# GatorSense/HyperPRI

Hardware: AMD Instinct MI355X
Metric: HSI cubes/sec (608x968x238) fwd+bwd (higher is better)
Workload: dtype f32; 1 GPU; CubeNET-64 n_channels=238 HSI 608x968 fp32, per-GPU batch 2, train mode, BCEWithLogits, fwd+bwd; global_batch=2, parallelism=dp1

## Files before the change

### hyperpri_amd/csrc/elementwise.hip

```cpp
#include "common.h"

static inline int ew_blocks(long long total) {
  long long b = (total + 255) / 256;
  if (b > 8192) b = 8192;
  if (b < 1) b = 1;
  return (int)b;
}

__global__ void nchw_to_nhwc_kernel(const float* __restrict__ src, float* __restrict__ dst, int C, long long P,
                                    int cs, int coff, int Cw) {
  __shared__ float tile[32][65];
  const int n = blockIdx.z;
  const long long p0 = (long long)blockIdx.x * 64;
  const int c0 = blockIdx.y * 32;
  const int tx = threadIdx.x & 63, ty = threadIdx.x >> 6;
  for (int r = ty; r < 32; r += 4) {
    const int c = c0 + r;
    const long long p = p0 + tx;
    tile[r][tx] = (c < C && p < P) ? src[((long long)n * C + c) * P + p] : 0.f;
  }
  __syncthreads();
  const int cx = threadIdx.x & 31, py = threadIdx.x >> 5;
  for (int r = py; r < 64; r += 8) {
    const long long p = p0 + r;
    const int c = c0 + cx;
    if (p < P && c < Cw) dst[((long long)n * P + p) * cs + coff + c] = tile[cx][r];
  }
}

__global__ __launch_bounds__(256) void nchw_to_nhwc_v4_kernel(const float* __restrict__ src, float* __restrict__ dst, int C,
                                                              long long P, int cs, int coff, int Cw, PlaneOut pl) {
  __shared__ float tile[128][65];
  const int n = blockIdx.z;
  const long long p0 = (long long)blockIdx.x * 128;
  const int c0 = blockIdx.y * 64;
  const int tx = threadIdx.x & 31, ty = threadIdx.x >> 5;
#pragma unroll
  for (int r = ty; r < 64; r += 8) {
    const int c = c0 + r;
    const long long p = p0 + tx * 4;
    f32x4 v = {0.f, 0.f, 0.f, 0.f};
    if (c < C && p < P) v = *reinterpret_cast<const f32x4*>(src + ((long long)n * C + c) * P + p);
    const int rc = (r + (tx >> 3)) & 63;
    tile[tx * 4 + 0][rc] = v[0]; tile[tx * 4 + 1][rc] = v[1]; tile[tx * 4 + 2][rc] = v[2]; tile[tx * 4 + 3][rc] = v[3];
  }
  __syncthreads();
  const int cq = threadIdx.x & 15, py = threadIdx.x >> 4;
#pragma unroll
  for (int r = py; r < 128; r += 16) {
    const long long p = p0 + r;
    const int c = c0 + cq * 4;
    if (p < P && (c < Cw || c < pl.cw)) {
      const int ro = r >> 5;
      f32x4 v = {tile[r][(cq * 4 + 0 + ro) & 63], tile[r][(cq * 4 + 1 + ro) & 63], tile[r][(cq * 4 + 2 + ro) & 63],
                 tile[r][(cq * 4 + 3 + ro) & 63]};
      if (dst != nullptr && c < Cw) *reinterpret_cast<f32x4*>(dst + ((long long)n * P + p) * cs + coff + c) = v;
      if (c < pl.cw) plane_store4(pl, (size_t)((long long)n * P + p), c, v[0], v[1], v[2], v[3]);
    }
  }
}

__global__ void nhwc_to_nchw_kernel(const float* __restrict__ src, float* __restrict__ dst, int C, long long P,
                                    int cs, int coff, int accumulate) {
  __shared__ float tile[64][33];
  const int n = blockIdx.z;
  const long long p0 = (long long)blockIdx.x * 64;
  const int c0 = blockIdx.y * 32;
  const int cx = threadIdx.x & 31, py = threadIdx.x >> 5;
  for (int r = py; r < 64; r += 8) {
    const long long p = p0 + r;
    const int c = c0 + cx;
    tile[r][cx] = (p < P && c < C) ? src[((long long)n * P + p) * cs + coff + c] : 0.f;
  }
  __syncthreads();
  const int tx = threadIdx.x & 63, ty = threadIdx.x >> 6;
  for (int r = ty; r < 32; r += 4) {
    const int c = c0 + r;
    const long long p = p0 + tx;
    if (c < C && p < P) {
      float* o = dst + ((long long)n * C + c) * P + p;
      *o = accumulate ? *o + tile[tx][r] : tile[tx][r];
    }
  }
}

template <bool B16>
__device__ __forceinline__ float4 ew_load4(const float* __restrict__ p) {
  if (B16) {
    const bf16x4_t v = *reinterpret_cast<const bf16x4_t*>(p);
    return make_float4((float)v[0], (float)v[1], (float)v[2], (float)v[3]);
  }
  return *reinterpret_cast<const float4*>(p);
}
template <bool B16>
__device__ __forceinline__ void ew_store4(float* __restrict__ p, float4 v) {
  if (B16) {
    bf16x4_t h;
    h[0] = (h16_t)v.x; h[1] = (h16_t)v.y; h[2] = (h16_t)v.z; h[3] = (h16_t)v.w;
    *reinterpret_cast<bf16x4_t*>(p) = h;
  } else {
    *reinterpret_cast<float4*>(p) = v;
  }
}
template <bool B16>
__device__ __forceinline__ const float* ew_at(const float* base, long long idx) {
  return B16 ? reinterpret_cast<const float*>(reinterpret_cast<const h16_t*>(base) + idx) : base + idx;
}
template <bool B16>
__device__ __forceinline__ float* ew_at(float* base, long long idx) {
  return B16 ? reinterpret_cast<float*>(reinterpret_cast<h16_t*>(base) + idx) : base + idx;
}

template <bool XB>
__global__ void maxpool2_fwd_kernel(const float* __restrict__ x, int x_cs, int x_coff, float* __restrict__ y, int y_cs,
                                    int y_coff, int N, int H, int W, int OH, int OW, int C4v, int C4, PlaneOut pl) {
  const long long total = (long long)N * OH * OW * C4;
  for (long long i = (long long)blockIdx.x * blockDim.x + threadIdx.x; i < total; i += (long long)gridDim.x * blockDim.x) {
    const int c = (int)(i % C4) * 4;
    long long r = i / C4;
    const int ox = (int)(r % OW); r /= OW;
    const int oy = (int)(r % OH);
    const int n = (int)(r / OH);
    const size_t opix = (size_t)(((long long)n * OH + oy) * OW + ox);
    if (c >= C4v * 4) { plane_store4(pl, opix, c, 0.f, 0.f, 0.f, 0.f); continue; }
    const long long b = (((long long)n * H + 2 * oy) * W + 2 * ox) * x_cs + x_coff + c;
    const float4 v00 = ew_load4<XB>(ew_at<XB>(x, b));
    const float4 v01 = ew_load4<XB>(ew_at<XB>(x, b + x_cs));
    const float4 v10 = ew_load4<XB>(ew_at<XB>(x, b + (long long)W * x_cs));
    const float4 v11 = ew_load4<XB>(ew_at<XB>(x, b + (long long)W * x_cs + x_cs));
    float4 m;
    m.x = fmaxf(fmaxf(v00.x, v01.x), fmaxf(v10.x, v11.x));
    m.y = fmaxf(fmaxf(v00.y, v01.y), fmaxf(v10.y, v11.y));
    m.z = fmaxf(fmaxf(v00.z, v01.z), fmaxf(v10.z, v11.z));
    m.w = fmaxf(fmaxf(v00.w, v01.w), fmaxf(v10.w, v11.w));
    if (y != nullptr) *reinterpret_cast<float4*>(y + opix * y_cs + y_coff + c) = m;
    if (pl.p != nullptr) plane_store4(pl, opix, c, m.x, m.y, m.z, m.w);
  }
}

__device__ __forceinline__ int first_argmax4(float a, float b, float c, float d) {
  int k = 0; float m = a;
  if (b > m) { m = b; k = 1; }
  if (c > m) { m = c; k = 2; }
  if (d > m) { k = 3; }
  return k;
}

template <bool XB, bool DXB>
__global__ void maxpool2_bwd_kernel(const float* __restrict__ x, int x_cs, int x_coff, const float* __restrict__ dy,
                                    int dy_cs, int dy_coff, float* __restrict__ dx, int dx_cs, int dx_coff, int N, int H,
                                    int W, int OH, int OW, int C4, int accumulate) {
  const int WH = (H + 1) >> 1, WW = (W + 1) >> 1;
  const unsigned total = (unsigned)N * WH * WW * C4;
  for (unsigned i = blockIdx.x * blockDim.x + threadIdx.x; i < total; i += gridDim.x * blockDim.x) {
    const unsigned c = (i % (unsigned)C4) * 4u;
    unsigned r = i / (unsigned)C4;
    const int wx = (int)(r % (unsigned)WW); r /= (unsigned)WW;
    const int wy = (int)(r % (unsigned)WH);
    const int n = (int)(r / (unsigned)WH);
    const int iy = 2 * wy, ix = 2 * wx;
    const bool row1 = iy + 1 < H, col1 = ix + 1 < W, pooled = wy < OH && wx < OW;
    const long long pix = ((long long)n * H + iy) * W + ix;
    float4 o[4] = {make_float4(0.f, 0.f, 0.f, 0.f), make_float4(0.f, 0.f, 0.f, 0.f), make_float4(0.f, 0.f, 0.f, 0.f),
                   make_float4(0.f, 0.f, 0.f, 0.f)};
    if (pooled) {
      const long long b = pix * x_cs + x_coff + c;
      const float4 v00 = ew_load4<XB>(ew_at<XB>(x, b));
      const float4 v01 = ew_load4<XB>(ew_at<XB>(x, b + x_cs));
      const float4 v10 = ew_load4<XB>(ew_at<XB>(x, b + (long long)W * x_cs));
      const float4 v11 = ew_load4<XB>(ew_at<XB>(x, b + (long long)W * x_cs + x_cs));
      const float4 g = *reinterpret_cast<const float4*>(dy + (((long long)n * OH + wy) * OW + wx) * dy_cs + dy_coff + c);
      const int kx = first_argmax4(v00.x, v01.x, v10.x, v11.x), ky = first_argmax4(v00.y, v01.y, v10.y, v11.y);
      const int kz = first_argmax4(v00.z, v01.z, v10.z, v11.z), kw = first_argmax4(v00.w, v01.w, v10.w, v11.w);
#pragma unroll
      for (int m = 0; m < 4; ++m) {
        o[m].x = kx == m ? g.x : 0.f; o[m].y = ky == m ? g.y : 0.f; o[m].z = kz == m ? g.z : 0.f; o[m].w = kw == m ? g.w : 0.f;
      }
    }
    const long long p = pix * dx_cs + dx_coff + c;
    float* pm[4] = {ew_at<DXB>(dx, p), ew_at<DXB>(dx, p + dx_cs), ew_at<DXB>(dx, p + (long long)W * dx_cs),
                    ew_at<DXB>(dx, p + (long long)W * dx_cs + dx_cs)};
    const bool ok[4] = {true, col1, row1, row1 && col1};
    if (accumulate) {
      float4 old[4];
#pragma unroll
      for (int m = 0; m < 4; ++m) old[m] = ok[m] ? ew_load4<DXB>(pm[m]) : make_float4(0.f, 0.f, 0.f, 0.f);
#pragma unroll
      for (int m = 0; m < 4; ++m) { o[m].x += old[m].x; o[m].y += old[m].y; o[m].z += old[m].z; o[m].w += old[m].w; }
    }
#pragma unroll
    for (int m = 0; m < 4; ++m)
      if (ok[m]) ew_store4<DXB>(pm[m], o[m]);
  }
}

__global__ void copy_slice_kernel(const float* __restrict__ s, int s_cs, int s_coff, float* __restrict__ d, int d_cs,
                                  int d_coff, long long P, int C4, int accumulate) {
  const long long total = P * C4;
  for (long long i = (long long)blockIdx.x * blockDim.x + threadIdx.x; i < total; i += (long long)gridDim.x * blockDim.x) {
    const long long p = i / C4;
    const int c = (int)(i - p * C4) * 4;
    float4 v = *reinterpret_cast<const float4*>(s + p * s_cs + s_coff + c);
    float* o = d + p * d_cs + d_coff + c;
    if (accumulate) {
      const float4 w = *reinterpret_cast<const float4*>(o);
      v.x += w.x; v.y += w.y; v.z += w.z; v.w += w.w;
    }
    *reinterpret_cast<float4*>(o) = v;
  }
}

__global__ void fill_pad_kernel(float* __restrict__ d, int cs, int coff, int N, int H, int W, int C4, int y0, int y1,
                                int x0, int x1) {
  const long long total = (long long)N * H * W * C4;
  for (long long i = (long long)blockIdx.x * blockDim.x + threadIdx.x; i < total; i += (long long)gridDim.x * blockDim.x) {
    const int c = (int)(i % C4) * 4;
    long long r = i / C4;
    const int ix = (int)(r % W); r /= W;
    const int iy = (int)(r % H);
    if (iy >= y0 && iy < y1 && ix >= x0 && ix < x1) continue;
    *reinterpret_cast<float4*>(d + (i / C4) * cs + coff + c) = make_float4(0.f, 0.f, 0.f, 0.f);
  }
}

__global__ void shift_copy_kernel(const float* __restrict__ s, int s_cs, int s_coff, int Hs, int Ws, float* __restrict__ d,
                                  int d_cs, int d_coff, int N, int Hd, int Wd, int oy, int ox, int C4, int accumulate) {
  const long long total = (long long)N * Hd * Wd * C4;
  for (long long i = (long long)blockIdx.x * blockDim.x + threadIdx.x; i < total; i += (long long)gridDim.x * blockDim.x) {
    const int c = (int)(i % C4) * 4;
    long long r = i / C4;
    const int ix = (int)(r % Wd); r /= Wd;
    const int iy = (int)(r % Hd);
    const int n = (int)(r / Hd);
    const int sy = iy - oy, sx = ix - ox;
    float4 v = make_float4(0.f, 0.f, 0.f, 0.f);
    if (sy >= 0 && sy < Hs && sx >= 0 && sx < Ws)
      v = *reinterpret_cast<const float4*>(s + (((long long)n * Hs + sy) * Ws + sx) * s_cs + s_coff + c);
    float* o = d + (i / C4) * d_cs + d_coff + c;
    if (accumulate) {
      const float4 w = *reinterpret_cast<const float4*>(o);
      v.x += w.x; v.y += w.y; v.z += w.z; v.w += w.w;
    }
    *reinterpret_cast<float4*>(o) = v;
  }
}

__global__ void fill_kernel(float* __restrict__ d, long long n, float v) {
  for (long long i = (long long)blockIdx.x * blockDim.x + threadIdx.x; i < n; i += (long long)gridDim.x * blockDim.x) d[i] = v;
}

typedef h16_t bf16x8 __attribute__((ext_vector_type(8)));
__device__ __forceinline__ float oc_bce_elem(float x, float y) { return fmaxf(x, 0.f) - x * y + log1pf(expf(-fabsf(x))); }
__device__ __forceinline__ float oc_bce_grad(float xi, float yi) {
  const float e = expf(-fabsf(xi)), r = 1.f / (1.f + e);
  const float sp = xi >= 0.f ? r : e * r, sn = xi >= 0.f ? e * r : r;
  return (1.f - yi) * sp - yi * sn;
}

template <bool XB>
__device__ __forceinline__ float4 oc_load4(const float* __restrict__ x, size_t idx) {
  if (XB) {
    const bf16x4_t v = *reinterpret_cast<const bf16x4_t*>(reinterpret_cast<const h16_t*>(x) + idx);
    return make_float4((float)v[0], (float)v[1], (float)v[2], (float)v[3]);
  }
  return *reinterpret_cast<const float4*>(x + idx);
}

template <bool BCE, bool XB>
__global__ __launch_bounds__(256) void outconv_fwd_kernel(const float* __restrict__ x, int x_cs, int x_coff, const float* __restrict__ w,
                                   const float* __restrict__ b, float* __restrict__ y, int N, long long P, int C, int K,
                                   const float* __restrict__ target, double* __restrict__ partial) {
  __shared__ double bred[256];
  double bsum = 0.0;
  const int gl = threadIdx.x & 15;
  const long long grp = ((long long)blockIdx.x * blockDim.x + threadIdx.x) >> 4;
  const long long ngrp = ((long long)gridDim.x * blockDim.x) >> 4;
  const int C4 = (C + 3) >> 2;
  if (!XB && K == 1 && (C & 3) == 0 && C4 <= 64) {
    float4 wq[4];
    int qi[4];
#pragma unroll
    for (int j = 0; j < 4; ++j) {
      const int q = gl + 16 * j;
      qi[j] = min(q, C4 - 1) * 4;
      wq[j] = q < C4 ? *reinterpret_cast<const float4*>(w + q * 4) : make_float4(0.f, 0.f, 0.f, 0.f);
    }
    const int nj = (C4 + 15) >> 4;
    const float b0 = b ? b[0] : 0.f;
    const long long NP = (long long)N * P;
    for (long long pg0 = grp; pg0 < NP; pg0 += 4 * ngrp) {
      float4 v[4][4];
#pragma unroll
      for (int u = 0; u < 4; ++u) {
        const long long pg = min(pg0 + u * ngrp, NP - 1);
        const float* xp = x + pg * x_cs + x_coff;
#pragma unroll
        for (int j = 0; j < 4; ++j)
          if (j < nj) v[u][j] = *reinterpret_cast<const float4*>(xp + qi[j]);
      }
      float mine = 0.f;
#pragma unroll
      for (int u = 0; u < 4; ++u) {
        float s = 0.f;
#pragma unroll
        for (int j = 0; j < 4; ++j)
          if (j < nj) { s += v[u][j].x * wq[j].x; s += v[u][j].y * wq[j].y; s += v[u][j].z * wq[j].z; s += v[u][j].w * wq[j].w; }
        s += __shfl_xor(s, 8, 16); s += __shfl_xor(s, 4, 16); s += __shfl_xor(s, 2, 16); s += __shfl_xor(s, 1, 16);
        if (gl == u) mine = s;
      }
      const long long pgm = pg0 + gl * ngrp;
      if (gl < 4 && pgm < NP) {
        const float o = mine + b0;
        y[pgm] = o;
        if (BCE) bsum += (double)oc_bce_elem(o, target[pgm]);
      }
    }
  } else
  for (long long pg = grp; pg < (long long)N * P; pg += ngrp) {
    for (int k = 0; k < K; ++k) {
      float s = 0.f;
      for (int q = gl; q < C4; q += 16) {
        const float4 v = oc_load4<XB>(x, (size_t)pg * x_cs + x_coff + q * 4);
        const float* wk = w + (long long)k * C + q * 4;
        s += v.x * wk[0];
        if (q * 4 + 1 < C) s += v.y * wk[1];
        if (q * 4 + 2 < C) s += v.z * wk[2];
        if (q * 4 + 3 < C) s += v.w * wk[3];
      }
      s += __shfl_xor(s, 8, 16); s += __shfl_xor(s, 4, 16); s += __shfl_xor(s, 2, 16); s += __shfl_xor(s, 1, 16);
      if (gl == 0) {
        const long long n = pg / P, p = pg - n * P;
        const float v = s + (b ? b[k] : 0.f);
        y[(n * K + k) * P + p] = v;
        if (BCE) bsum += (double)oc_bce_elem(v, target[(n * K + k) * P + p]);
      }
    }
  }
  if (BCE) {
    bred[threadIdx.x] = bsum;
    __syncthreads();
    for (int wd = 128; wd > 0; wd >>= 1) {
      if (threadIdx.x < wd) bred[threadIdx.x] += bred[threadIdx.x + wd];
      __syncthreads();
    }
    if (threadIdx.x == 0) partial[blockIdx.x] = bred[0];
  }
}

__device__ __forceinline__ float oc_mul_then_add(float a, float b, float s) {
#pragma clang fp contract(off)
  const float p = a * b;
  return s + p;
}

template <bool BCE, int NJ>
__global__ __launch_bounds__(256) void bn_outconv_fwd_kernel(const float* __restrict__ x, int x_cs, int x_coff, const float* __restrict__ scale,
                                                             const float* __restrict__ shift, int relu, const float* __restrict__ w,
                                                             const float* __restrict__ b, float* __restrict__ y, long long NP, int C,
                                                             const float* __restrict__ target, double* __restrict__ partial) {
  __shared__ double bred[256];
  double bsum = 0.0;
// ... 356 lines not shown
#pragma unroll
    for (int u = 0; u < UF; ++u) add(g[u], xv[u]);
  }
  for (; p < p1; p += rows) {
    float g = dy[p];
    if (BCE) g = oc_bce_grad(g, target[p]) * gs;
    const float4 xq = live ? *reinterpret_cast<const float4*>(x + p * x_cs + x_coff + c) : make_float4(0.f, 0.f, 0.f, 0.f);
    add(g, xq);
  }
  red[0][threadIdx.x] = make_float4(s1[0], s1[1], s1[2], s1[3]);
  red[1][threadIdx.x] = make_float4(s2[0], s2[1], s2[2], s2[3]);
  red[2][threadIdx.x] = make_float4(sw[0], sw[1], sw[2], sw[3]);
  redb[threadIdx.x] = sb;
  __syncthreads();
  if (pr == 0) {
    float4 t1 = make_float4(0.f, 0.f, 0.f, 0.f), t2 = t1, t3 = t1;
    float tb = 0.f;
    for (int r = 0; r < rows; ++r) {
      const float4 a = red[0][r * CQ + cq], b = red[1][r * CQ + cq], d = red[2][r * CQ + cq];
      t1.x += a.x; t1.y += a.y; t1.z += a.z; t1.w += a.w;
      t2.x += b.x; t2.y += b.y; t2.z += b.z; t2.w += b.w;
      t3.x += d.x; t3.y += d.y; t3.z += d.z; t3.w += d.w;
      tb += redb[r * CQ + cq];
    }
    float* o = bnpart + ((size_t)blockIdx.x * 2) * Cpart + c;
    *reinterpret_cast<float4*>(o) = t1;
    *reinterpret_cast<float4*>(o + Cpart) = t2;
    float* h = hwpart + ((size_t)blockIdx.x * 2) * Cpart;
    *reinterpret_cast<float4*>(h + c) = t3;
    if (blockIdx.y == 0 && cq == 0) h[Cpart] = tb;
  }
}

template <bool BCE>
__global__ __launch_bounds__(256) void bn_head_apply_kernel(const float* __restrict__ dy, const float* __restrict__ target,
                                                            const float* __restrict__ gscale, float lscale, const float* __restrict__ x,
                                                            int x_cs, int x_coff, const float* __restrict__ w, float* __restrict__ dx,
                                                            int dx_cs, int dx_coff, const float* __restrict__ mean,
                                                            const float* __restrict__ invstd, const float* __restrict__ scale,
                                                            const float* __restrict__ shift, const float* __restrict__ sums, int NP, int C,
                                                            int Cw, int CQ, int relu, int use_batch_stats, float* __restrict__ dxpart,
                                                            int Cpart) {
  const float gs = BCE ? (gscale ? gscale[0] : 1.f) / (float)((double)NP) * lscale : 1.f;
  __shared__ float4 red[256];
  const int rows = 256 / CQ;
  const int cq = threadIdx.x % CQ, pr = threadIdx.x / CQ;
  const int c = (blockIdx.y * CQ + cq) * 4;
  const bool live = c < Cw;
  float acc[4] = {0.f, 0.f, 0.f, 0.f};
  const float inv_np = 1.f / (float)NP;
  float sc[4], sh[4], mu[4], is[4], k1[4], k2[4], wv[4];
#pragma unroll
  for (int j = 0; j < 4; ++j) {
    const bool ok = c + j < C;
    sc[j] = ok ? scale[c + j] : 0.f;
    sh[j] = ok ? shift[c + j] : 0.f;
    mu[j] = ok ? mean[c + j] : 0.f;
    is[j] = ok ? invstd[c + j] : 0.f;
    wv[j] = ok ? w[c + j] : 0.f;
    k1[j] = (ok && use_batch_stats) ? sums[c + j] * inv_np : 0.f;
    k2[j] = (ok && use_batch_stats) ? sums[C + c + j] * inv_np : 0.f;
  }
  auto put = [&](long long q, float gl, const float4& xq) {
    const float xx[4] = {xq.x, xq.y, xq.z, xq.w};
    float o[4];
#pragma unroll
    for (int j = 0; j < 4; ++j) {
      const float gv = 0.f + gl * wv[j];
      const float gj = (!relu || (xx[j] * sc[j] + sh[j] > 0.f)) ? gv : 0.f;
      const float xh = (xx[j] - mu[j]) * is[j];
      o[j] = (c + j < C) ? sc[j] * (gj - k1[j] - xh * k2[j]) : 0.f;
      acc[j] += o[j];
    }
    *reinterpret_cast<float4*>(dx + (size_t)q * dx_cs + dx_coff + c) = make_float4(o[0], o[1], o[2], o[3]);
  };
  const long long per = ((long long)NP + gridDim.x - 1) / gridDim.x;
  const long long q0 = (long long)blockIdx.x * per;
  const long long q1 = (q0 + per < NP) ? q0 + per : NP;
  long long q = q0 + pr;
  for (; q + 3 * rows < q1; q += 4 * rows) {
    float g[4];
    float4 xv[4];
#pragma unroll
    for (int u = 0; u < 4; ++u) {
      const long long pg = q + u * rows;
      g[u] = dy[pg];
      if (BCE && CQ < 4) g[u] = oc_bce_grad(g[u], target[pg]) * gs;
      xv[u] = live ? *reinterpret_cast<const float4*>(x + (size_t)pg * x_cs + x_coff + c) : make_float4(0.f, 0.f, 0.f, 0.f);
    }
    if (BCE && CQ >= 4) {
      float lg = 0.f, lt = 0.f;
#pragma unroll
      for (int u = 0; u < 4; ++u)
        if (cq == u) { lg = g[u]; lt = target[q + u * rows]; }
      const float mine = oc_bce_grad(lg, lt) * gs;
#pragma unroll
      for (int u = 0; u < 4; ++u) g[u] = __shfl(mine, (threadIdx.x & 63 & ~(CQ - 1)) + u, 64);
    }
    if (live) {
#pragma unroll
      for (int u = 0; u < 4; ++u) put(q + u * rows, g[u], xv[u]);
    }
  }
  if (live)
    for (; q < q1; q += rows) {
      float g = dy[q];
      if (BCE) g = oc_bce_grad(g, target[q]) * gs;
      put(q, g, *reinterpret_cast<const float4*>(x + (size_t)q * x_cs + x_coff + c));
    }
  if (dxpart != nullptr) {
    red[threadIdx.x] = make_float4(acc[0], acc[1], acc[2], acc[3]);
    __syncthreads();
    if (pr == 0 && c < Cpart) {
      float4 t = make_float4(0.f, 0.f, 0.f, 0.f);
      for (int r = 0; r < rows; ++r) { const float4 a = red[r * CQ + cq]; t.x += a.x; t.y += a.y; t.z += a.z; t.w += a.w; }
      float* o = dxpart + ((size_t)blockIdx.x * 2) * Cpart + c;
      *reinterpret_cast<float4*>(o) = t;
      *reinterpret_cast<float4*>(o + Cpart) = make_float4(0.f, 0.f, 0.f, 0.f);
    }
  }
}

template <bool APPLY>
__global__ __launch_bounds__(256) void bn_pool_bwd_kernel(const float* __restrict__ dskip, int ds_cs, int ds_coff,
                                                          const float* __restrict__ dpool, int dp_cs, int dp_coff,
                                                          const float* __restrict__ x, int x_cs, int x_coff, float* __restrict__ dx,
                                                          int dx_cs, int dx_coff, const float* __restrict__ mean,
                                                          const float* __restrict__ invstd, const float* __restrict__ scale,
                                                          const float* __restrict__ shift, const float* __restrict__ sums, int N, int H,
                                                          int W, int C, int Cw, int CQ, float* __restrict__ part, int Cpart) {
  __shared__ float4 red[2][256];
  const int rows = 256 / CQ;
  const int cq = threadIdx.x % CQ, pr = threadIdx.x / CQ;
  const int c = (blockIdx.y * CQ + cq) * 4;
  const int WH = (H + 1) >> 1, WW = (W + 1) >> 1, OH = H >> 1, OW = W >> 1;
  const unsigned nwin = (unsigned)N * WH * WW;
  const unsigned per = (nwin + gridDim.x - 1) / gridDim.x;
  const unsigned w0 = blockIdx.x * per;
  const unsigned w1 = min(nwin, w0 + per);
  float s1[4] = {0.f, 0.f, 0.f, 0.f}, s2[4] = {0.f, 0.f, 0.f, 0.f};
  if (c < (APPLY ? Cw : C)) {
    const float inv_np = 1.f / (float)(N * H * W);
    float sc[4], sh[4], mu[4], is[4], k1[4], k2[4];
#pragma unroll
    for (int j = 0; j < 4; ++j) {
      const bool ok = c + j < C;
      sc[j] = ok ? scale[c + j] : 0.f;
      sh[j] = ok ? shift[c + j] : 0.f;
      mu[j] = ok ? mean[c + j] : 0.f;
      is[j] = ok ? invstd[c + j] : 0.f;
      k1[j] = (ok && APPLY) ? sums[c + j] * inv_np : 0.f;
      k2[j] = (ok && APPLY) ? sums[C + c + j] * inv_np : 0.f;
    }
    for (unsigned wi = w0 + pr; wi < w1; wi += rows) {
      const int wx = (int)(wi % (unsigned)WW);
      const unsigned r = wi / (unsigned)WW;
      const int wy = (int)(r % (unsigned)WH), n = (int)(r / (unsigned)WH);
      const int iy = 2 * wy, ix = 2 * wx;
      const bool row1 = iy + 1 < H, col1 = ix + 1 < W, pooled = wy < OH && wx < OW;
      const long long pix = ((long long)n * H + iy) * W + ix;
#define HPRI_WIN_OK(m_) ((((m_) & 1) == 0 || col1) && (((m_) >> 1) == 0 || row1))
#define HPRI_WIN_PIX(m_) (pix + ((m_) & 1) + (long long)((m_) >> 1) * W)
      float4 xv[4], dv[4];
#pragma unroll
      for (int m = 0; m < 4; ++m) {
        xv[m] = HPRI_WIN_OK(m) ? *reinterpret_cast<const float4*>(x + HPRI_WIN_PIX(m) * x_cs + x_coff + c) : make_float4(0.f, 0.f, 0.f, 0.f);
        dv[m] = (dskip != nullptr && HPRI_WIN_OK(m)) ? *reinterpret_cast<const float4*>(dskip + HPRI_WIN_PIX(m) * ds_cs + ds_coff + c) : make_float4(0.f, 0.f, 0.f, 0.f);
      }
      const float4 gp = pooled ? *reinterpret_cast<const float4*>(dpool + (((long long)n * OH + wy) * OW + wx) * dp_cs + dp_coff + c) : make_float4(0.f, 0.f, 0.f, 0.f);
      const float gq[4] = {gp.x, gp.y, gp.z, gp.w};
      float xx[4][4], dd[4][4], o[4][4];
#pragma unroll
      for (int m = 0; m < 4; ++m) {
        xx[m][0] = xv[m].x; xx[m][1] = xv[m].y; xx[m][2] = xv[m].z; xx[m][3] = xv[m].w;
        dd[m][0] = dv[m].x; dd[m][1] = dv[m].y; dd[m][2] = dv[m].z; dd[m][3] = dv[m].w;
      }
#pragma unroll
      for (int j = 0; j < 4; ++j) {
        float y[4];
#pragma unroll
        for (int m = 0; m < 4; ++m) y[m] = (c + j < C) ? fmaxf(xx[m][j] * sc[j] + sh[j], 0.f) : 0.f;
        const int k = first_argmax4(y[0], y[1], y[2], y[3]);
#pragma unroll
        for (int m = 0; m < 4; ++m) {
          float g = (pooled && k == m) ? gq[j] : 0.f;
          if (dskip != nullptr) g += dd[m][j];
          const float gj = (y[m] > 0.f) ? g : 0.f;
          const float xh = (xx[m][j] - mu[j]) * is[j];
          if (APPLY) {
            o[m][j] = (c + j < C) ? sc[j] * (gj - k1[j] - xh * k2[j]) : 0.f;
          } else if (HPRI_WIN_OK(m)) {
            s1[j] += gj;
            s2[j] += gj * xh;
          }
        }
      }
      if (APPLY) {
#pragma unroll
        for (int m = 0; m < 4; ++m)
          if (HPRI_WIN_OK(m)) *reinterpret_cast<float4*>(dx + HPRI_WIN_PIX(m) * dx_cs + dx_coff + c) = make_float4(o[m][0], o[m][1], o[m][2], o[m][3]);
      }
#undef HPRI_WIN_OK
#undef HPRI_WIN_PIX
    }
  }
  if (!APPLY) {
    red[0][threadIdx.x] = make_float4(s1[0], s1[1], s1[2], s1[3]);
    red[1][threadIdx.x] = make_float4(s2[0], s2[1], s2[2], s2[3]);
    __syncthreads();
    if (pr == 0 && c < Cpart) {
      float4 t1 = make_float4(0.f, 0.f, 0.f, 0.f), t2 = t1;
      for (int r = 0; r < rows; ++r) {
        const float4 a = red[0][r * CQ + cq], b = red[1][r * CQ + cq];
        t1.x += a.x; t1.y += a.y; t1.z += a.z; t1.w += a.w;
        t2.x += b.x; t2.y += b.y; t2.z += b.z; t2.w += b.w;
      }
      float* o = part + ((size_t)blockIdx.x * 2) * Cpart + c;
      *reinterpret_cast<float4*>(o) = t1;
      *reinterpret_cast<float4*>(o + Cpart) = t2;
    }
  }
}

__global__ __launch_bounds__(256) void bn_apply_relu_pool_kernel(const float* __restrict__ x, int x_cs, int x_coff, float* __restrict__ y,
                                                                 int y_cs, int y_coff, float* __restrict__ pool, int p_cs, int p_coff,
                                                                 const float* __restrict__ scale, const float* __restrict__ shift, int N,
                                                                 int H, int W, int C, int C4, int relu) {
  const int WH = (H + 1) >> 1, WW = (W + 1) >> 1, OH = H >> 1, OW = W >> 1;
  const unsigned total = (unsigned)N * WH * WW * C4;
  for (unsigned i = blockIdx.x * blockDim.x + threadIdx.x; i < total; i += gridDim.x * blockDim.x) {
    const int c = (int)(i % (unsigned)C4) * 4;
    unsigned r = i / (unsigned)C4;
    const int wx = (int)(r % (unsigned)WW); r /= (unsigned)WW;
    const int wy = (int)(r % (unsigned)WH);
    const int n = (int)(r / (unsigned)WH);
    const int iy = 2 * wy, ix = 2 * wx;
    const bool row1 = iy + 1 < H, col1 = ix + 1 < W, pooled = wy < OH && wx < OW;
    const long long pix = ((long long)n * H + iy) * W + ix;
    float sc[4], sh[4];
#pragma unroll
    for (int j = 0; j < 4; ++j) {
      const bool ok = c + j < C;
      sc[j] = ok ? scale[c + j] : 0.f;
      sh[j] = ok ? shift[c + j] : 0.f;
    }
    float4 v[4], o[4];
#pragma unroll
    for (int m = 0; m < 4; ++m) {
      const bool okm = ((m & 1) == 0 || col1) && ((m >> 1) == 0 || row1);
      v[m] = okm ? *reinterpret_cast<const float4*>(x + (pix + (m & 1) + (long long)(m >> 1) * W) * x_cs + x_coff + c) : make_float4(0.f, 0.f, 0.f, 0.f);
    }
#pragma unroll
    for (int m = 0; m < 4; ++m) {
      o[m].x = (c + 0 < C) ? v[m].x * sc[0] + sh[0] : 0.f; o[m].y = (c + 1 < C) ? v[m].y * sc[1] + sh[1] : 0.f;
      o[m].z = (c + 2 < C) ? v[m].z * sc[2] + sh[2] : 0.f; o[m].w = (c + 3 < C) ? v[m].w * sc[3] + sh[3] : 0.f;
      if (relu) { o[m].x = fmaxf(o[m].x, 0.f); o[m].y = fmaxf(o[m].y, 0.f); o[m].z = fmaxf(o[m].z, 0.f); o[m].w = fmaxf(o[m].w, 0.f); }
      const bool okm = ((m & 1) == 0 || col1) && ((m >> 1) == 0 || row1);
      if (okm) *reinterpret_cast<float4*>(y + (pix + (m & 1) + (long long)(m >> 1) * W) * y_cs + y_coff + c) = o[m];
    }
    if (pooled) {
      float4 mx;
      mx.x = fmaxf(fmaxf(o[0].x, o[1].x), fmaxf(o[2].x, o[3].x));
      mx.y = fmaxf(fmaxf(o[0].y, o[1].y), fmaxf(o[2].y, o[3].y));
      mx.z = fmaxf(fmaxf(o[0].z, o[1].z), fmaxf(o[2].z, o[3].z));
      mx.w = fmaxf(fmaxf(o[0].w, o[1].w), fmaxf(o[2].w, o[3].w));
      *reinterpret_cast<float4*>(pool + (((long long)n * OH + wy) * OW + wx) * p_cs + p_coff + c) = mx;
    }
  }
}

__device__ __forceinline__ float synth_u(unsigned long long seed, unsigned long long idx) {
  unsigned long long z = seed * 0x9E3779B97F4A7C15ull + idx;
  z ^= z >> 30; z *= 0xBF58476D1CE4E5B9ull;
  z ^= z >> 27; z *= 0x94D049BB133111EBull;
  z ^= z >> 31;
  return (float)(z >> 40) * (1.0f / 16777216.0f);
}

__global__ void synth_kernel(float* __restrict__ d, long long n, unsigned long long seed, int mode, float thr, float scale) {
  for (long long i = (long long)blockIdx.x * blockDim.x + threadIdx.x; i < n; i += (long long)gridDim.x * blockDim.x) {
    const float u = synth_u(seed, (unsigned long long)i);
    d[i] = mode == 0 ? u : (mode == 1 ? (u > thr ? 1.f : 0.f) : (2.f * u - 1.f) * scale);
  }
}

extern "C" int hpri_nchw_to_nhwc_pl(const float* src, float* dst, int N, int C, long long P, int cs, int coff, int Cw,
                                    void* planes, long long plane_stride, int pl_cs, int pl_coff, int pl_cw, int npl,
                                    hipStream_t stream);
extern "C" int hpri_maxpool2_fwd_pl(const float* x, int x_cs, int x_coff, float* y, int y_cs, int y_coff, int N, int H,
                                    int W, int C, void* planes, long long plane_stride, int pl_cs, int pl_coff, int pl_cw,
                                    int npl, hipStream_t stream);
extern "C" int hpri_nchw_to_nhwc(const float* src, float* dst, int N, int C, long long P, int cs, int coff, int Cw,
                                 hipStream_t stream) {
  return hpri_nchw_to_nhwc_pl(src, dst, N, C, P, cs, coff, Cw, nullptr, 0, 0, 0, 0, 0, stream);
}

extern "C" int hpri_nchw_to_nhwc_pl(const float* src, float* dst, int N, int C, long long P, int cs, int coff, int Cw,
                                    void* planes, long long plane_stride, int pl_cs, int pl_coff, int pl_cw, int npl,
                                    hipStream_t stream) {
  HPRI_REQUIRE(src && (dst || planes) && N > 0 && C > 0 && P > 0 && Cw >= C && Cw + coff <= cs, "nchw_to_nhwc: bad arguments");
  PlaneOut po;
  { const int rc_ = hpri_plane_out(&po, planes, plane_stride, pl_cs, pl_coff, pl_cw, npl, C); if (rc_ != HPRI_OK) return rc_; }
  if (P % 4 == 0 && cs % 4 == 0 && coff % 4 == 0 && Cw % 4 == 0 && ((uintptr_t)src & 15) == 0 && ((uintptr_t)dst & 15) == 0) {
    dim3 grid4((unsigned)hpri_cdiv64(P, 128), (unsigned)hpri_cdiv(Cw > po.cw ? Cw : po.cw, 64), (unsigned)N);
    hipLaunchKernelGGL(nchw_to_nhwc_v4_kernel, grid4, dim3(256), 0, stream, src, dst, C, P, cs, coff, Cw, po);
    HPRI_CHECK_LAUNCH();
    return HPRI_OK;
  }
  if (planes != nullptr || dst == nullptr) return hpri_set_error(HPRI_ERR_UNSUPPORTED, "nchw_to_nhwc_pl: plane output needs the 16-byte aligned form");
  dim3 grid((unsigned)hpri_cdiv64(P, 64), (unsigned)hpri_cdiv(Cw, 32), (unsigned)N);
  hipLaunchKernelGGL(nchw_to_nhwc_kernel, grid, dim3(256), 0, stream, src, dst, C, P, cs, coff, Cw);
  HPRI_CHECK_LAUNCH();
  return HPRI_OK;
}

extern "C" int hpri_nhwc_to_nchw(const float* src, float* dst, int N, int C, long long P, int cs, int coff,
                                 int accumulate, hipStream_t stream) {
  HPRI_REQUIRE(src && dst && N > 0 && C > 0 && P > 0 && C + coff <= cs, "nhwc_to_nchw: bad arguments");
  dim3 grid((unsigned)hpri_cdiv64(P, 64), (unsigned)hpri_cdiv(C, 32), (unsigned)N);
  hipLaunchKernelGGL(nhwc_to_nchw_kernel, grid, dim3(256), 0, stream, src, dst, C, P, cs, coff, accumulate);
  HPRI_CHECK_LAUNCH();
  return HPRI_OK;
}

#define HPRI_REQ_V4(cs, coff) HPRI_REQUIRE((cs) % 4 == 0 && (coff) % 4 == 0, "channel stride/offset must be multiples of 4")

extern "C" int hpri_maxpool2_fwd(const float* x, int x_cs, int x_coff, float* y, int y_cs, int y_coff, int N, int H,
                                 int W, int C, hipStream_t stream) {
  return hpri_maxpool2_fwd_pl(x, x_cs, x_coff, y, y_cs, y_coff, N, H, W, C, nullptr, 0, 0, 0, 0, 0, stream);
}

template <bool XB>
static int maxpool2_fwd_impl(const float* x, int x_cs, int x_coff, float* y, int y_cs, int y_coff, int N, int H,
                             int W, int C, void* planes, long long plane_stride, int pl_cs, int pl_coff, int pl_cw,
                             int npl, hipStream_t stream) {
  HPRI_REQUIRE(x && (y || planes) && N > 0 && H >= 2 && W >= 2 && C > 0 && C % 4 == 0, "maxpool2_fwd: bad arguments");
  HPRI_REQ_V4(x_cs, x_coff);
  if (y != nullptr) { HPRI_REQ_V4(y_cs, y_coff); }
  PlaneOut po;
  { const int rc_ = hpri_plane_out(&po, planes, plane_stride, pl_cs, pl_coff, pl_cw, npl, C); if (rc_ != HPRI_OK) return rc_; }
  const int OH = H / 2, OW = W / 2;
  const int c4 = (C > po.cw ? C : po.cw) / 4;
  hipLaunchKernelGGL(maxpool2_fwd_kernel<XB>, dim3(ew_blocks((long long)N * OH * OW * c4)), dim3(256), 0, stream, x, x_cs,
                     x_coff, y, y_cs, y_coff, N, H, W, OH, OW, C / 4, c4, po);
  HPRI_CHECK_LAUNCH();
  return HPRI_OK;
}

extern "C" int hpri_maxpool2_fwd_pl(const float* x, int x_cs, int x_coff, float* y, int y_cs, int y_coff, int N, int H,
                                    int W, int C, void* planes, long long plane_stride, int pl_cs, int pl_coff, int pl_cw,
                                    int npl, hipStream_t stream) {
  HPRI_REQUIRE(y != nullptr, "maxpool2_fwd: bad arguments");
  return maxpool2_fwd_impl<false>(x, x_cs, x_coff, y, y_cs, y_coff, N, H, W, C, planes, plane_stride, pl_cs, pl_coff, pl_cw, npl, stream);
}

extern "C" int hpri_maxpool2_fwd_x16(const void* x16, int x_cs, int x_coff, float* y, int y_cs, int y_coff, int N, int H,
                                     int W, int C, void* planes, long long plane_stride, int pl_cs, int pl_coff, int pl_cw,
                                     int npl, hipStream_t stream) {
  return maxpool2_fwd_impl<true>(reinterpret_cast<const float*>(x16), x_cs, x_coff, y, y_cs, y_coff, N, H, W, C, planes, plane_stride,
                                 pl_cs, pl_coff, pl_cw, npl, stream);
}

extern "C" int hpri_maxpool2_bwd(const float* x, int x_cs, int x_coff, const float* dy, int dy_cs, int dy_coff, float* dx,
                                 int dx_cs, int dx_coff, int N, int H, int W, int C, int accumulate, hipStream_t stream) {
  HPRI_REQUIRE(x && dy && dx && N > 0 && H >= 2 && W >= 2 && C > 0 && C % 4 == 0, "maxpool2_bwd: bad arguments");
  HPRI_REQ_V4(x_cs, x_coff); HPRI_REQ_V4(dy_cs, dy_coff); HPRI_REQ_V4(dx_cs, dx_coff);
  const long long windows = (long long)N * ((H + 1) / 2) * ((W + 1) / 2) * (C / 4);
  HPRI_REQUIRE(windows < (1ll << 31), "maxpool2_bwd: more than 2^31 window quads");
  hipLaunchKernelGGL((maxpool2_bwd_kernel<false, false>), dim3(ew_blocks(windows)), dim3(256), 0, stream, x, x_cs,
                     x_coff, dy, dy_cs, dy_coff, dx, dx_cs, dx_coff, N, H, W, H / 2, W / 2, C / 4, accumulate);
  HPRI_CHECK_LAUNCH();
  return HPRI_OK;
}

extern "C" int hpri_maxpool2_bwd_x16(const void* x, int x_bf16, int x_cs, int x_coff, const float* dy, int dy_cs, int dy_coff, void* dx,
                                     int dx_bf16, int dx_cs, int dx_coff, int N, int H, int W, int C, int accumulate, hipStream_t stream) {
  HPRI_REQUIRE(x && dy && dx && N > 0 && H >= 2 && W >= 2 && C > 0 && C % 4 == 0, "maxpool2_bwd_x16: bad arguments");
  HPRI_REQ_V4(x_cs, x_coff); HPRI_REQ_V4(dy_cs, dy_coff); HPRI_REQ_V4(dx_cs, dx_coff);
  const long long windows = (long long)N * ((H + 1) / 2) * ((W + 1) / 2) * (C / 4);
  HPRI_REQUIRE(windows < (1ll << 31), "maxpool2_bwd_x16: more than 2^31 window quads");
  const float* xf = reinterpret_cast<const float*>(x);
  float* dxf = reinterpret_cast<float*>(dx);
#define HPRI_MP_BWD(XB_, DXB_)                                                                                              \
  hipLaunchKernelGGL((maxpool2_bwd_kernel<XB_, DXB_>), dim3(ew_blocks(windows)), dim3(256), 0, stream, xf, x_cs, x_coff, dy, \
                     dy_cs, dy_coff, dxf, dx_cs, dx_coff, N, H, W, H / 2, W / 2, C / 4, accumulate)
  if (x_bf16 && dx_bf16) HPRI_MP_BWD(true, true);
  else if (x_bf16) HPRI_MP_BWD(true, false);
  else if (dx_bf16) HPRI_MP_BWD(false, true);
  else HPRI_MP_BWD(false, false);
#undef HPRI_MP_BWD
  HPRI_CHECK_LAUNCH();
  return HPRI_OK;
}

extern "C" int hpri_copy_slice(const float* src, int s_cs, int s_coff, float* dst, int d_cs, int d_coff, long long P,
                               int C, int accumulate, hipStream_t stream) {
  HPRI_REQUIRE(src && dst && P > 0 && C > 0 && C % 4 == 0, "copy_slice: bad arguments");
  HPRI_REQ_V4(s_cs, s_coff); HPRI_REQ_V4(d_cs, d_coff);
  hipLaunchKernelGGL(copy_slice_kernel, dim3(ew_blocks(P * (C / 4))), dim3(256), 0, stream, src, s_cs, s_coff, dst, d_cs,
                     d_coff, P, C / 4, accumulate);
  HPRI_CHECK_LAUNCH();
  return HPRI_OK;
}

extern "C" int hpri_shift_copy(const float* src, int s_cs, int s_coff, int Hs, int Ws, float* dst, int d_cs, int d_coff, int N,
                               int Hd, int Wd, int oy, int ox, int C, int accumulate, hipStream_t stream) {
  HPRI_REQUIRE(src && dst && N > 0 && Hs > 0 && Ws > 0 && Hd > 0 && Wd > 0 && C > 0 && C % 4 == 0, "shift_copy: bad arguments");
  HPRI_REQ_V4(s_cs, s_coff); HPRI_REQ_V4(d_cs, d_coff);
  hipLaunchKernelGGL(shift_copy_kernel, dim3(ew_blocks((long long)N * Hd * Wd * (C / 4))), dim3(256), 0, stream, src, s_cs,
                     s_coff, Hs, Ws, dst, d_cs, d_coff, N, Hd, Wd, oy, ox, C / 4, accumulate);
  HPRI_CHECK_LAUNCH();
  return HPRI_OK;
}

extern "C" int hpri_fill_pad(float* dst, int cs, int coff, int N, int H, int W, int C, int y0, int y1, int x0, int x1,
                             hipStream_t stream) {
  HPRI_REQUIRE(dst && N > 0 && H > 0 && W > 0 && C > 0 && C % 4 == 0, "fill_pad: bad arguments");
  HPRI_REQ_V4(cs, coff);
  hipLaunchKernelGGL(fill_pad_kernel, dim3(ew_blocks((long long)N * H * W * (C / 4))), dim3(256), 0, stream, dst, cs, coff, N,
                     H, W, C / 4, y0, y1, x0, x1);
  HPRI_CHECK_LAUNCH();
  return HPRI_OK;
}

extern "C" int hpri_fill(float* dst, long long n, float value, hipStream_t stream) {
  HPRI_REQUIRE(dst && n > 0, "fill: bad arguments");
  hipLaunchKernelGGL(fill_kernel, dim3(ew_blocks(n)), dim3(256), 0, stream, dst, n, value);
  HPRI_CHECK_LAUNCH();
  return HPRI_OK;
}

template <bool XB>
static int outconv_fwd_impl(const float* x, int x_cs, int x_coff, const float* w, const float* b, float* y, const float* target,
                            double* partial, size_t partial_doubles, int N, long long P, int C, int K, hipStream_t stream) {
  constexpr int VEC = XB ? 8 : 4;
  HPRI_REQUIRE(x && w && y && N > 0 && P > 0 && C > 0 && K > 0, "outconv_fwd: bad arguments");
  HPRI_REQUIRE(x_cs % 4 == 0 && x_coff % 4 == 0, "outconv_fwd: channel stride / offset must be multiples of 4");
  HPRI_REQUIRE(((C + 3) / 4) * 4 + x_coff <= x_cs, "outconv_fwd: channel stride too small for 4-channel reads");
  const int nb = ew_blocks((long long)N * P * 16);
  if (target != nullptr && (size_t)nb > partial_doubles) return hpri_set_error(HPRI_ERR_WORKSPACE, "outconv_fwd_bce: partial buffer too small");
  const int Cr = ((C + 16 * VEC - 1) / (16 * VEC)) * (16 * VEC);
  const bool wide = K == 1 && (XB || C > 256 || (C & 3) != 0) && Cr <= 12288 && x_cs % VEC == 0 && x_coff % VEC == 0 &&
                    ((C + VEC - 1) / VEC) * VEC + x_coff <= x_cs;
  if (wide) {
    if (target != nullptr)
      hipLaunchKernelGGL((outconv_fwd_wide_kernel<true, XB>), dim3(nb), dim3(256), Cr * sizeof(float), stream, x, x_cs, x_coff, w, b, y,
                         (long long)N * P, C, target, partial);
    else
      hipLaunchKernelGGL((outconv_fwd_wide_kernel<false, XB>), dim3(nb), dim3(256), Cr * sizeof(float), stream, x, x_cs, x_coff, w, b, y,
                         (long long)N * P, C, (const float*)nullptr, (double*)nullptr);
  } else if (target != nullptr) {
    hipLaunchKernelGGL((outconv_fwd_kernel<true, XB>), dim3(nb), dim3(256), 0, stream, x, x_cs, x_coff, w, b, y, N, P, C, K, target, partial);
  } else {
    hipLaunchKernelGGL((outconv_fwd_kernel<false, XB>), dim3(nb), dim3(256), 0, stream, x, x_cs, x_coff, w, b, y, N, P, C, K,
                       (const float*)nullptr, (double*)nullptr);
  }
  HPRI_CHECK_LAUNCH();
  return HPRI_OK;
}

extern "C" int hpri_outconv_fwd(const float* x, int x_cs, int x_coff, const float* w, const float* b, float* y, int N,
                                long long P, int C, int K, hipStream_t stream) {
  return outconv_fwd_impl<false>(x, x_cs, x_coff, w, b, y, nullptr, nullptr, 0, N, P, C, K, stream);
}

extern "C" size_t hpri_outconv_fwd_bce_blocks(int N, long long P) { return (size_t)ew_blocks((long long)N * P * 16); }
extern "C" int hpri_outconv_fwd_bce(const float* x, int x_cs, int x_coff, const float* w, const float* b, float* y, const float* target,
                                    double* partial, size_t partial_doubles, int N, long long P, int C, int K, hipStream_t stream) {
  HPRI_REQUIRE(target && partial, "outconv_fwd_bce: bad arguments");
  return outconv_fwd_impl<false>(x, x_cs, x_coff, w, b, y, target, partial, partial_doubles, N, P, C, K, stream);
}

extern "C" int hpri_outconv_fwd_x16(const void* x16, int x_cs, int x_coff, const float* w, const float* b, float* y, const float* target,
                                    double* partial, size_t partial_doubles, int N, long long P, int C, int K, hipStream_t stream) {
  HPRI_REQUIRE(target == nullptr || partial != nullptr, "outconv_fwd_x16: bad arguments");
  return outconv_fwd_impl<true>(reinterpret_cast<const float*>(x16), x_cs, x_coff, w, b, y, target, partial, partial_doubles, N, P, C, K, stream);
}

static inline int pick_cq(int c4) { int q = 1; while (q < c4 && q < 64) q <<= 1; return q; }

extern "C" int hpri_outconv_bwd_plan(int N, long long P, int C, int K, int* nblk, int* Cpart) {
  const int c4 = hpri_cdiv(C, 4), cq = pick_cq(c4), rows = 256 / cq, ycols = hpri_cdiv(c4, cq);
  long long nb = 1024 / ((long long)ycols * K);
  const long long maxb = ((long long)N * P + rows * 8 - 1) / (rows * 8);
  if (nb > maxb) nb = maxb;
  if (nb < 1) nb = 1;
  *nblk = (int)nb; *Cpart = ycols * cq * 4;
  return HPRI_OK;
}

template <bool XB>
static int outconv_bwd_impl(const float* dy, const float* target, const float* gscale, const float* x, int x_cs, int x_coff,
                            const float* w, float* dx, int dx_cs, int dx_coff, int dx_cw, int dx_accumulate, float* dw, float* db,
                            int accumulate_param_grads, float* workspace, size_t ws_floats, int N, long long P, int C,
                            int K, hipStream_t stream, int dx_bf16 = 0) {
  const bool bce = target != nullptr;
  HPRI_REQUIRE(dy && x && w && dw && workspace && N > 0 && P > 0 && C > 0 && K > 0, "outconv_bwd: bad arguments");
  HPRI_REQ_V4(x_cs, x_coff);
  if (dx != nullptr) {
    HPRI_REQ_V4(dx_cs, dx_coff);
    HPRI_REQUIRE(dx_cw % 4 == 0 && dx_cw >= C && dx_cw + dx_coff <= dx_cs, "outconv_bwd: dx channel layout");
    dim3 grid(ew_blocks((long long)N * P * (dx_cw / 4)));
    int dq = 1;
    if (K == 1) {
      dq = pick_cq(dx_cw / 4);
      const int ycols = hpri_cdiv(dx_cw / 4, dq), rows = 256 / dq;
      long long nbx = hpri_cdiv((long long)N * P, (long long)rows * 4);
      const long long cap = 8192 / ycols > 0 ? 8192 / ycols : 1;
      if (nbx > cap) nbx = cap;
      grid = dim3((unsigned)nbx, ycols);
    }
    HPRI_REQUIRE(!dx_bf16 || K == 1, "outconv_bwd: a bf16 input gradient is built for one class");
    if (dx_bf16 && bce)
      hipLaunchKernelGGL((outconv_bwd_data_kernel<true, true>), grid, dim3(256), 0, stream, dy, w,
                         dx, dx_cs, dx_coff, N, P, C, dx_cw, K, dx_accumulate, target, gscale, dq, hpri_loss_scale());
    else if (dx_bf16)
      hipLaunchKernelGGL((outconv_bwd_data_kernel<false, true>), grid, dim3(256), 0, stream, dy, w,
                         dx, dx_cs, dx_coff, N, P, C, dx_cw, K, dx_accumulate, (const float*)nullptr, (const float*)nullptr, dq, hpri_loss_scale());
    else if (bce)
      hipLaunchKernelGGL(outconv_bwd_data_kernel<true>, grid, dim3(256), 0, stream, dy, w,
                         dx, dx_cs, dx_coff, N, P, C, dx_cw, K, dx_accumulate, target, gscale, dq, hpri_loss_scale());
    else
      hipLaunchKernelGGL(outconv_bwd_data_kernel<false>, grid, dim3(256), 0, stream, dy, w,
                         dx, dx_cs, dx_coff, N, P, C, dx_cw, K, dx_accumulate, (const float*)nullptr, (const float*)nullptr, dq, hpri_loss_scale());
    HPRI_CHECK_LAUNCH();
  }
  int nblk, Cpart;
  hpri_outconv_bwd_plan(N, P, C, K, &nblk, &Cpart);
  if ((size_t)nblk * K * 2 * Cpart > ws_floats) return hpri_set_error(HPRI_ERR_WORKSPACE, "outconv_bwd: workspace too small");
  const int c4 = hpri_cdiv(C, 4), cq = pick_cq(c4);
  if (bce)
    hipLaunchKernelGGL((outconv_bwd_weight_kernel<true, XB>), dim3(nblk, hpri_cdiv(c4, cq), K), dim3(256), 0, stream, dy, x, x_cs, x_coff,
                       N, P, C, K, cq, workspace, Cpart, target, gscale, hpri_loss_scale());
  else
    hipLaunchKernelGGL((outconv_bwd_weight_kernel<false, XB>), dim3(nblk, hpri_cdiv(c4, cq), K), dim3(256), 0, stream, dy, x, x_cs, x_coff,
                       N, P, C, K, cq, workspace, Cpart, (const float*)nullptr, (const float*)nullptr, hpri_loss_scale());
  HPRI_CHECK_LAUNCH();
  hipLaunchKernelGGL(outconv_bwd_weight_finalize_kernel, dim3(K * (C + 1)), dim3(256), 0, stream, workspace,
                     nblk, K, Cpart, C, dw, db, accumulate_param_grads);
  HPRI_CHECK_LAUNCH();
  return HPRI_OK;
}

extern "C" int hpri_outconv_bwd(const float* dy, const float* x, int x_cs, int x_coff, const float* w, float* dx,
                                int dx_cs, int dx_coff, int dx_cw, int dx_accumulate, float* dw, float* db,
                                int accumulate_param_grads, float* workspace, size_t ws_floats, int N, long long P, int C,
                                int K, hipStream_t stream) {
  return outconv_bwd_impl<false>(dy, nullptr, nullptr, x, x_cs, x_coff, w, dx, dx_cs, dx_coff, dx_cw, dx_accumulate, dw, db,
                          accumulate_param_grads, workspace, ws_floats, N, P, C, K, stream);
}

extern "C" int hpri_outconv_bwd_bce(const float* logits, const float* target, const float* gscale, const float* x, int x_cs, int x_coff,
                                    const float* w, float* dx, int dx_cs, int dx_coff, int dx_cw, int dx_accumulate, float* dw,
                                    float* db, int accumulate_param_grads, float* workspace, size_t ws_floats, int N, long long P,
                                    int C, int K, hipStream_t stream) {
  HPRI_REQUIRE(target != nullptr, "outconv_bwd_bce: null target");
  return outconv_bwd_impl<false>(logits, target, gscale, x, x_cs, x_coff, w, dx, dx_cs, dx_coff, dx_cw, dx_accumulate, dw, db,
                                 accumulate_param_grads, workspace, ws_floats, N, P, C, K, stream);
}

extern "C" int hpri_outconv_bwd_x16(const float* dy, const float* target, const float* gscale, const void* x16, int x_cs, int x_coff,
                                    const float* w, void* dx, int dx_bf16, int dx_cs, int dx_coff, int dx_cw, int dx_accumulate, float* dw,
                                    float* db, int accumulate_param_grads, float* workspace, size_t ws_floats, int N, long long P,
                                    int C, int K, hipStream_t stream) {
  return outconv_bwd_impl<true>(dy, target, gscale, reinterpret_cast<const float*>(x16), x_cs, x_coff, w, reinterpret_cast<float*>(dx),
                                dx_cs, dx_coff, dx_cw, dx_accumulate, dw, db, accumulate_param_grads, workspace, ws_floats, N, P, C, K,
                                stream, dx_bf16);
}

extern "C" int hpri_col_finalize(const float* part, int nblk, int Cpart, int C, float* sums, float* out1, float* out2,
                                 int accumulate, float* zero_out, hipStream_t stream);

static inline size_t rup4(size_t v) { return (v + 3) & ~(size_t)3; }

extern "C" int hpri_bn_relu_outconv_fwd(const float* x, int x_cs, int x_coff, const float* scale, const float* shift, int relu,
                                        const float* w, const float* b, float* y, const float* target, double* partial,
                                        size_t partial_doubles, int N, long long P, int C, hipStream_t stream) {
  HPRI_REQUIRE(x && scale && shift && w && y && N > 0 && P > 0 && C > 0 && C <= 256, "bn_relu_outconv_fwd: bad arguments");
  HPRI_REQUIRE(target == nullptr || partial != nullptr, "bn_relu_outconv_fwd: a target needs the partial buffer");
  HPRI_REQ_V4(x_cs, x_coff);
  HPRI_REQUIRE(((C + 3) / 4) * 4 + x_coff <= x_cs, "bn_relu_outconv_fwd: channel stride too small for 4-channel reads");
  const int nb = ew_blocks((long long)N * P * 16);
  if (target != nullptr && (size_t)nb > partial_doubles) return hpri_set_error(HPRI_ERR_WORKSPACE, "bn_relu_outconv_fwd: partial buffer too small");
  const int nj = (((C + 3) >> 2) + 15) >> 4;
#define HPRI_BOF(BCE_, NJ_)                                                                                                        \
  hipLaunchKernelGGL((bn_outconv_fwd_kernel<BCE_, NJ_>), dim3(nb), dim3(256), 0, stream, x, x_cs, x_coff, scale, shift, relu, w, b, y, \
                     (long long)N * P, C, target, partial)
  if (target != nullptr) { if (nj == 1) HPRI_BOF(true, 1); else if (nj == 2) HPRI_BOF(true, 2); else HPRI_BOF(true, 4); }
  else { if (nj == 1) HPRI_BOF(false, 1); else if (nj == 2) HPRI_BOF(false, 2); else HPRI_BOF(false, 4); }
#undef HPRI_BOF
  HPRI_CHECK_LAUNCH();
  return HPRI_OK;
}

extern "C" size_t hpri_bn_relu_outconv_bwd_ws(int N, long long P, int C) {
  int nblk, Cpart;
  hpri_outconv_bwd_plan(N, P, C, 1, &nblk, &Cpart);
  return 3 * (size_t)nblk * 2 * Cpart + 2 * rup4(2 * (size_t)C);
}

extern "C" int hpri_bn_relu_outconv_bwd(const float* dy, const float* target, const float* gscale, const float* x, int x_cs, int x_coff,
                                        const float* w, float* dx, int dx_cs, int dx_coff, int Cw, const float* mean,
                                        const float* invstd, const float* scale, const float* shift, float* dgamma, float* dbeta,
                                        int accumulate_bn_grads, float* dbias, int accumulate_dbias, float* dw, float* db,
                                        int accumulate_head_grads, float* workspace, size_t ws_floats, int N, long long P, int C,
                                        int relu, int use_batch_stats, hipStream_t stream) {
// ... 342 lines not shown
```

Measured before the change: 69.31 cubes/s.

## Add persistent pipelined row-tiled NCHW-to-NHWC transpose with swizzled LDS

Adds a persistent NCHW-to-NHWC transpose kernel for the dense non-plane case. Each block loops over pixel runs and channel blocks, prefetching the next tile's vector loads into registers while it stores the current tile. The LDS tile uses an XOR swizzle to avoid bank conflicts, and the grid is sized from the CU count. The aim is to hide global load latency and write full NHWC rows, at the cost of more registers per thread and reduced occupancy.

```diff
diff --git a/hyperpri_amd/csrc/elementwise.hip b/hyperpri_amd/csrc/elementwise.hip
--- a/hyperpri_amd/csrc/elementwise.hip
+++ b/hyperpri_amd/csrc/elementwise.hip
@@ -57,6 +57,71 @@
       if (dst != nullptr && c < Cw) *reinterpret_cast<f32x4*>(dst + ((long long)n * P + p) * cs + coff + c) = v;
       if (c < pl.cw) plane_store4(pl, (size_t)((long long)n * P + p), c, v[0], v[1], v[2], v[3]);
     }
+  }
+}
+
+template <int PX, int CHB>
+struct LayoutMap {
+  static constexpr int QP = PX / 4, QC = CHB / 4, L = PX * CHB / 1024;
+  __host__ __device__ static void load_item(int t, int i, int* cq, int* e, int* pq) {
+    const int j = i * 64 + (t >> 2);
+    *e = t & 3; *pq = j % QP; *cq = j / QP;
+  }
+  __host__ __device__ static int slot(int pl, int cq) { return pl * QC + (cq ^ ((pl >> 2) & 7)); }
+  __host__ __device__ static void store_item(int t, int i, int* r, int* q) {
+    const int idx = i * 256 + t;
+    *q = idx % QC; *r = idx / QC;
+  }
+};
+
+template <int PX, int CHB>
+__global__ __launch_bounds__(256) void nchw_to_nhwc_rows_kernel(const float* __restrict__ src, float* __restrict__ dst, int C,
+                                                                long long P, int cs, int coff, int Cw, int ncb, int runs) {
+  using M = LayoutMap<PX, CHB>;
+  constexpr int L = M::L;
+  __shared__ f32x4 tile[PX * M::QC];
+  float* tilef = reinterpret_cast<float*>(tile);
+  const int t = threadIdx.x, n = blockIdx.y;
+  const float* sn = src + (long long)n * C * P;
+  float* dn = dst + (long long)n * P * cs + coff;
+  int run = blockIdx.x, cb = 0;
+  if (run >= runs) return;
+  f32x4 v[L];
+  auto issue = [&](int run_, int cb_) {
+#pragma unroll
+    for (int i = 0; i < L; ++i) {
+      int cq, e, pq;
+      M::load_item(t, i, &cq, &e, &pq);
+      const int c = cb_ * CHB + cq * 4 + e;
+      const long long p = (long long)run_ * PX + pq * 4;
+      v[i] = f32x4{0.f, 0.f, 0.f, 0.f};
+      if (c < C && p < P) v[i] = *reinterpret_cast<const f32x4*>(sn + (long long)c * P + p);
+    }
+  };
+  issue(run, cb);
+  for (;;) {
+    const int crun = run, ccb = cb;
+#pragma unroll
+    for (int i = 0; i < L; ++i) {
+      int cq, e, pq;
+      M::load_item(t, i, &cq, &e, &pq);
+#pragma unroll
+      for (int k = 0; k < 4; ++k) tilef[M::slot(pq * 4 + k, cq) * 4 + e] = v[i][k];
+    }
+    if (++cb == ncb) { cb = 0; run += gridDim.x; }
+    const bool more = run < runs;
+    if (more) issue(run, cb);
+    __syncthreads();
+#pragma unroll
+    for (int i = 0; i < L; ++i) {
+      int r, q;
+      M::store_item(t, i, &r, &q);
+      const long long p = (long long)crun * PX + r;
+      const int c = ccb * CHB + q * 4;
+      if (p < P && c < Cw) *reinterpret_cast<f32x4*>(dn + p * cs + c) = tile[M::slot(r, q)];
+    }
+    if (!more) break;
+    __syncthreads();
   }
 }
 
@@ -1019,6 +1084,21 @@
   PlaneOut po;
   { const int rc_ = hpri_plane_out(&po, planes, plane_stride, pl_cs, pl_coff, pl_cw, npl, C); if (rc_ != HPRI_OK) return rc_; }
   if (P % 4 == 0 && cs % 4 == 0 && coff % 4 == 0 && Cw % 4 == 0 && ((uintptr_t)src & 15) == 0 && ((uintptr_t)dst & 15) == 0) {
+    if (po.cw == 0 && dst != nullptr && hpri_cdiv64(P, 64) < (1ll << 30) && N <= 65535) {
+#define HPRI_ROWS(PX_, CHB_, WG_)                                                                                             \
+  {                                                                                                                           \
+    const int runs = (int)hpri_cdiv64(P, PX_), ncb = hpri_cdiv(Cw, CHB_);                                                       \
+    int gx = hpri_cdiv(WG_ * hpri_cu_count(), N);                                                                               \
+    if (gx > runs) gx = runs;                                                                                                 \
+    hipLaunchKernelGGL((nchw_to_nhwc_rows_kernel<PX_, CHB_>), dim3(gx, N), dim3(256), 0, stream, src, dst, C, P, cs, coff, Cw, \
+                       ncb, runs);                                                                                            \
+  }
+      if (Cw > 128) HPRI_ROWS(64, 256, 2)
+      else HPRI_ROWS(128, 64, 4)
+#undef HPRI_ROWS
+      HPRI_CHECK_LAUNCH();
+      return HPRI_OK;
+    }
     dim3 grid4((unsigned)hpri_cdiv64(P, 128), (unsigned)hpri_cdiv(Cw > po.cw ? Cw : po.cw, 64), (unsigned)N);
     hipLaunchKernelGGL(nchw_to_nhwc_v4_kernel, grid4, dim3(256), 0, stream, src, dst, C, P, cs, coff, Cw, po);
     HPRI_CHECK_LAUNCH();
```

New measurement: 69.58 cubes/s, median of 6. Within noise of the previous version (+0.4%).
